# hidayetersindursun/LangSplatV2

Measured on AMD Instinct MI355X. Metric: frames/s fwd+bwd @ 1M Gaussians 1080p 3+16ch; achieved HBM GB/s, higher is better.
Workload: dtype f32; 1 GPU; BASELINE cfg3: 1M Gaussians, 1920x1080, SH deg 3 + 16 dense language channels, fwd+bwd, all inputs require grad; 1 view per GPU; gaussians=1000000, width=1920, height=1080, lang_dim=16, sh_degree=3, global_batch=1, parallelism=single GPU

## Files before the change

langsplatv2_amd/csrc/render_bwd.hip:

```cpp
#include "render_common.h"
#include "render_det.h"

#ifndef LSR_BWD_SPLAT_PF
#define LSR_BWD_SPLAT_PF 1
#endif
#ifndef LSR_BWD_LO_RREG
#define LSR_BWD_LO_RREG 1
#endif
#ifndef LSR_BWD16_WAVES
#define LSR_BWD16_WAVES 4
#endif
#ifndef LSR_MF_WAVES
#define LSR_MF_WAVES 2
#endif

namespace lsr {

#define LSR_ORD_NB 64
#ifndef LSR_ORD_THREADS
#define LSR_ORD_THREADS 1024
#endif
#define LSR_ORD_KPT 16
__global__ void __launch_bounds__(LSR_ORD_THREADS) k_bwd_order(const uint32_t* __restrict__ lcount,
                                                    const uint32_t* __restrict__ tile_start, int n,
                                                    uint4* __restrict__ border)
{
    __shared__ uint32_t cnt[LSR_ORD_NB];
    const int q = n / 8, r = n % 8, x = blockIdx.x;
    const int lo = x < r ? x * (q + 1) : r * (q + 1) + (x - r) * q;
    const int len = q + (x < r ? 1 : 0);
    const int tid = threadIdx.x;
    if (tid < LSR_ORD_NB) cnt[tid] = 0u;
    __syncthreads();
    auto key = [&](int i) { return min((int)((lcount[lo + i] + 15u) >> 4), LSR_ORD_NB - 1); };
    constexpr int STEP = LSR_ORD_THREADS * LSR_ORD_KPT;
    int kr[LSR_ORD_KPT];
    for (int c = 0; c < len; c += STEP) {
#pragma unroll
        for (int j = 0; j < LSR_ORD_KPT; j++) {
            const int i = c + tid + LSR_ORD_THREADS * j;
            kr[j] = i < len ? key(i) : -1;
        }
#pragma unroll
        for (int j = 0; j < LSR_ORD_KPT; j++)
            if (kr[j] >= 0) atomicAdd(&cnt[kr[j]], 1u);
    }
    __syncthreads();
    if (tid < 64) {
        static_assert(LSR_ORD_NB == 64, "one bucket per lane");
        const uint32_t v = cnt[63 - tid];
        uint32_t incl = v;
#pragma unroll
        for (int d = 1; d < 64; d <<= 1) {
            const uint32_t u = __shfl_up(incl, d, 64);
            if (tid >= d) incl += u;
        }
        cnt[63 - tid] = (uint32_t)lo + incl - v;
    }
    __syncthreads();
    for (int c = 0; c < len; c += STEP) {
        if (len > STEP) {
#pragma unroll
            for (int j = 0; j < LSR_ORD_KPT; j++) {
                const int i = c + tid + LSR_ORD_THREADS * j;
                kr[j] = i < len ? key(i) : -1;
            }
        }
#pragma unroll
        for (int j = 0; j < LSR_ORD_KPT; j++)
            if (kr[j] >= 0) {
                const uint32_t blk = (uint32_t)(lo + c + tid + LSR_ORD_THREADS * j);
                border[atomicAdd(&cnt[kr[j]], 1u)] =
                    make_uint4(blk, tile_start[blk >> 2], tile_start[(blk >> 2) + 1], lcount[blk]);
            }
    }
}

hipError_t launch_bwd_order(const RenderArgs& a, uint4* border, hipStream_t st)
{
    const int n = 4 * a.cam.gx * a.cam.gy;
    if (n == 0) return hipSuccess;
    k_bwd_order<<<8, LSR_ORD_THREADS, 0, st>>>(a.lcount, a.tile_start, n, border);
    return hipGetLastError();
}

int grad_row_width(int D)
{
    const int nl = lang_set_for(D);
    const int nv = LSR_GROW_LANG + (nl > 0 ? nl : 0);
    return (nv + 31) / 32 * 32;
}

template <int NL>
struct BwdFrags {
    static constexpr int C = 3 + NL;
    static constexpr int KS = (C + 3) / 4;
    static constexpr int NBC = (C + 15) / 16;
    float dotB[KS][4];
    float chB[NBC][16];
    float momB[16];
};

template <int NL>
__device__ __forceinline__ float gd_at(const RenderBwdArgs& b, int c, int q, int bx, int by)
{
    const Cam& cm = b.f.cam;
    const int qx = bx + (q & 7), qy = by + (q >> 3);
    const bool ok = qx < cm.W && qy < cm.H && c < 3 + b.f.D;
    const size_t HW = (size_t)cm.H * cm.W;
    const size_t pix = (size_t)min(qy, cm.H - 1) * cm.W + min(qx, cm.W - 1);
    const float* src = c < 3 ? b.dout_color + (size_t)c * HW : b.dout_lang + (size_t)min(c - 3, max(b.f.D - 1, 0)) * HW;
    if (c >= 3 && b.f.D == 0) src = b.dout_color;
    const float v = src[pix];
    return ok ? v : 0.f;
}

#ifndef LSR_GRP_STRIDE
#define LSR_GRP_STRIDE 66
#endif
#define LSR_BUF_OOB 0x7ffffffc
#define LSR_MOM9_STRIDE 12
#define LSR_LOG2E 1.4426950408889634f
#define LSR_MF_ATOMIC(ptr, v) atomicAdd((ptr), (v))

__device__ __forceinline__ uint64_t lanes_abs_lt(float v, float bound)
{
    uint64_t m;
    asm("v_cmp_gt_f32_e64 %0, %1, |%2|" : "=s"(m) : "s"(bound), "v"(v));
    return m;
}

struct WaveStageG {
    float4 A[80];
    float4 B[80];
    uint32_t gid[80];
};

#define LSR_LST_CHUNK 16
struct WaveStageL {
    float4 A[2 * LSR_LST_CHUNK];
    float4 B[2 * LSR_LST_CHUNK];
};
template <int NL, bool LD, bool LST, bool DET = false>
constexpr int bwd_waves() { return (LST && LD && NL == 16 && !DET) ? LSR_BWD16_WAVES : LSR_MF_WAVES; }

__device__ __forceinline__ void glds16(const void* g, const void* lds)
{
    const uint32_t l = (uint32_t)(uintptr_t)lds;
    uint32_t keep;
    asm volatile("s_mov_b32 %0, m0\n\ts_mov_b32 m0, %2\n\ts_nop 0\n\tglobal_load_lds_dwordx4 %1, off\n\ts_mov_b32 m0, %0"
                 : "=&s"(keep) : "v"(g), "s"(l) : "memory");
}

template <int N>
__device__ __forceinline__ void wait_vmcnt()
{
    static_assert(N >= 0 && N <= 63, "vmcnt is 6 bits");
    asm volatile("s_waitcnt vmcnt(%0)" ::"n"(N) : "memory");
}

__device__ __forceinline__ int stage_candidates_geo(WaveStageG& st, int carry, bool valid, uint32_t gid, int pos,
                                                    int bx, int by, const float4* __restrict__ splatA,
                                                    const float4* __restrict__ splatB)
{
    float4 A = make_float4(0.f, 0.f, 0.f, 0.f), B = A;
    if (valid) {
        A = splatA[gid];
        B = splatB[gid];
    }
    const bool ok = valid && block_overlap(A.x, A.y, __float_as_uint(B.w), bx, by) &&
                    block_overlap_exact(A.x, A.y, A.z, A.w, B.x, B.z, bx, by);
    const uint64_t m = wave_ballot(ok);
    if (ok) {
        const int r = carry + __builtin_amdgcn_mbcnt_hi((uint32_t)(m >> 32), __builtin_amdgcn_mbcnt_lo((uint32_t)m, 0u));
        st.A[r] = A;
        st.B[r] = make_float4(B.x, B.y, B.z, __int_as_float(pos));
        st.gid[r] = gid;
    }
    wave_lds_fence();
    return __popcll(m);
}

__device__ __forceinline__ int stage_candidates_geo_rec(WaveStageG& st, int carry, bool valid, uint32_t gid, int pos,
                                                        int bx, int by, float4 A, float4 B)
{
    const bool ok = valid && block_overlap(A.x, A.y, __float_as_uint(B.w), bx, by) &&
                    block_overlap_exact(A.x, A.y, A.z, A.w, B.x, B.z, bx, by);
    const uint64_t m = wave_ballot(ok);
    if (ok) {
        const int r = carry + __builtin_amdgcn_mbcnt_hi((uint32_t)(m >> 32), __builtin_amdgcn_mbcnt_lo((uint32_t)m, 0u));
        st.A[r] = A;
        st.B[r] = make_float4(B.x, B.y, B.z, __int_as_float(pos));
        st.gid[r] = gid;
    }
    wave_lds_fence();
    return __popcll(m);
}

template <int NL>
__device__ __forceinline__ float feature_at(const RenderArgs& a, uint32_t gid, int c)
{
    const bool ok = c < 3 + a.D;
    const float* src = c < 3 ? a.rgb + 3 * (size_t)gid + c
                             : (ok ? a.lang + (size_t)gid * a.D + (c - 3) : a.rgb + 3 * (size_t)gid);
    const float v = *src;
    return ok ? v : 0.f;
}

template <int NL, bool VEC>
__device__ __forceinline__ int dot_channel(int t, int lg)
{
    if constexpr (VEC) {
        if (t < NL / 4) return 3 + 16 * (t >> 2) + 4 * lg + (t & 3);
        return lg < 3 ? lg : 3 + NL;
    }
    return 4 * t + lg;
}

template <int NL, bool VEC, int KS>
__device__ __forceinline__ void dot_features(const RenderArgs& a, uint32_t gid, int lg, float (&af)[KS])
{
    if constexpr (VEC) {
        static_assert(NL % 16 == 0 && KS == NL / 4 + 1, "VEC: whole 16-channel lines");
        const float4* row = reinterpret_cast<const float4*>(a.lang) + (size_t)gid * (NL / 4) + lg;
#pragma unroll
        for (int r = 0; r < NL / 16; r++) {
            const float4 v = row[4 * r];
            af[4 * r + 0] = v.x;
            af[4 * r + 1] = v.y;
            af[4 * r + 2] = v.z;
            af[4 * r + 3] = v.w;
        }
        const float c = a.rgb[3 * (size_t)gid + min(lg, 2)];
        af[NL / 4] = lg < 3 ? c : 0.f;
    } else {
#pragma unroll
        for (int t = 0; t < KS; t++) af[t] = feature_at<NL>(a, gid, 4 * t + lg);
    }
}

#define BWD_MFMA(a, b_, c) __builtin_amdgcn_mfma_f32_16x16x4f32((a), (b_), (c), 0, 0, 0)


template <int NL, bool LO = false, bool LD = false, bool SP = false, bool LST = false, bool DET = false>
__global__ void __launch_bounds__(64) __attribute__((amdgpu_waves_per_eu(bwd_waves<NL, LD, LST, DET>()))) k_render_bwd_mf(RenderBwdArgs b)
{
    static_assert(!(LST && SP), "the sparse-input backward follows the quick forward (no lists)");
    static_assert(!(DET && SP), "the deterministic backward expands the sparse input (lsr_api backward_quick)");
    static_assert(!LO || NL > 0, "language-only backward needs D > 0");
    static_assert(!SP || LO, "the sparse-input gradient is a language-only backward");
    static_assert(!LD || (!LO && NL % 16 == 0), "direct dL/dlang needs whole 16-channel lines");
    using FR = BwdFrags<NL>;
    constexpr int KS = FR::KS;
    constexpr bool VEC = LD;
    constexpr bool RREG = LD || (LO && !SP && LSR_BWD_LO_RREG);
    constexpr int NBC = (NL + 15) / 16;
    constexpr int NBA = NBC > 0 ? NBC : 1;
    __shared__ float2 sRG[64];
    __shared__ float sBc[64];
    constexpr int GS = LSR_GRP_STRIDE;
    __shared__ std::conditional_t<LST, WaveStageL, WaveStageG> stv;
    auto& st = stv;
    auto& stl = stv;
    constexpr int GCOL0 = LO ? 0 : (LD ? 16 : LSR_GROW_LANG);
    constexpr int GRL = (GCOL0 + NL + 15) / 16;
    constexpr int GRS = 16 * GRL + 4;
    constexpr int DUG = (16 * GS > 16 * GRS) ? 16 * GS : 16 * GRS;
    __shared__ float sDU[DUG];
    __shared__ __attribute__((aligned(16))) float sAT[16 * GS];
    static_assert(16 * LSR_MOM9_STRIDE <= 16 * GS, "moment rows must fit the aT tile");
    float* const sGr = sDU;
    float* const sMom = sAT;

    const RenderArgs& a = b.f;
    const Cam& c = a.cam;
    const WaveTile wt(a, LST ? a.border : nullptr);
    const int lane = threadIdx.x;
    const int lg = lane >> 4, li = lane & 15;
    const PixMap pm(c, wt.tile, lane + (wt.sub << 6));
    const bool inside = pm.px < c.W && pm.py < c.H;
    const float pfx = (float)pm.px, pfy = (float)pm.py;
    const float cx = (float)pm.bx + 3.5f, cy = (float)pm.by + 3.5f;
    const uint32_t rs = wt.ent ? wt.rs : a.tile_start[wt.tile];
    const size_t HW = (size_t)c.H * c.W;
    const size_t pix = (size_t)pm.py * c.W + pm.px;
    const int D = a.D;
    const int VP = b.VP;
    const float ddelx_dx = 0.5f * (float)c.W, ddely_dy = 0.5f * (float)c.H;
    const uint64_t nbg = (uint64_t)a.P * (uint64_t)VP * 4u;
    const uint64_t nbl = LD ? (uint64_t)a.P * (uint64_t)D * 4u : 0u;
    const bool buf_atom = nbg < (uint64_t)LSR_BUF_OOB && nbl < (uint64_t)LSR_BUF_OOB;
    const __amdgpu_buffer_rsrc_t rg =
        __builtin_amdgcn_make_buffer_rsrc(b.grad_acc, 0, (int)min(nbg, (uint64_t)LSR_BUF_OOB), 0x00020000);
    const __amdgpu_buffer_rsrc_t rl = __builtin_amdgcn_make_buffer_rsrc(
        LD ? b.lang_acc : b.grad_acc, 0, (int)min(LD ? nbl : nbg, (uint64_t)LSR_BUF_OOB), 0x00020000);

    const float T_final = inside ? a.final_T[pix] : 0.f;
    const int last = inside ? (int)a.n_contrib[pix] : 0;
    const int wmax = wave_max_i(last);
    if (wmax == 0) return;
    constexpr bool SPF = LSR_BWD_SPLAT_PF && NL <= 32;
    auto pl_at = [&](int q) -> uint32_t { const uint32_t v = a.point_list[rs + max(q, 0)]; return q >= 0 ? v : 0u; };
    uint32_t gid1 = 0u, gid2 = 0u;
    float4 A1 = make_float4(0.f, 0.f, 0.f, 0.f), B1 = A1;
    const uint32_t lcnt = LST ? (wt.ent ? wt.lc : a.lcount[4 * wt.tile + wt.sub]) : 0u;
    const size_t lbase = LST ? (size_t)4 * rs + (size_t)wt.sub * ((wt.ent ? wt.re : a.tile_start[wt.tile + 1]) - rs) : 0;
    if constexpr (!LST) {
        gid1 = pl_at(wmax - 1 - lane);
        if constexpr (SPF) {
            gid2 = pl_at(wmax - 65 - lane);
            A1 = a.splatA[gid1];
            B1 = a.splatB[gid1];
        }
        for (int e = lane; e < 80; e += 64) {
            st.A[e] = make_float4(0.f, 0.f, 0.f, 0.f);
            st.B[e] = make_float4(0.f, 0.f, 0.f, __int_as_float(0x7fffffff));
            st.gid[e] = 0u;
        }
    }
    auto list_dma = [&](int c0, int off) {
        const int e = (int)lcnt - 1 - (c0 + lane);
        const size_t src = lbase + (size_t)(e >= 0 ? e : 0);
        if (lane < LSR_LST_CHUNK) {
            glds16(a.listA + src, stl.A + off);
            glds16(a.listB + src, stl.B + off);
        }
    };

    float dr0 = 0.f, dr1 = 0.f, dr2 = 0.f;
    if constexpr (!LO) {
        dr0 = gd_at<NL>(b, 0, lane, pm.bx, pm.by);
        dr1 = gd_at<NL>(b, 1, lane, pm.bx, pm.by);
        dr2 = gd_at<NL>(b, 2, lane, pm.bx, pm.by);
    }
    float dotB[KS][4], chB[NBA][16];
    const uint64_t HW4 = (uint64_t)HW * 4u;
    const bool gd_buf = VEC && HW4 * (uint64_t)(D > 3 ? D : 3) < 0x7fffffffull;
    if (VEC && gd_buf) {
        const __amdgpu_buffer_rsrc_t rcol = __builtin_amdgcn_make_buffer_rsrc((void*)b.dout_color, 0, (int)(HW4 * 3u), 0x00020000);
        const __amdgpu_buffer_rsrc_t rlng = __builtin_amdgcn_make_buffer_rsrc((void*)b.dout_lang, 0, (int)(HW4 * (uint64_t)D), 0x00020000);
        const uint32_t hw4 = (uint32_t)HW4;
        auto poff = [&](int q) -> uint32_t {
            const int qx = pm.bx + (q & 7), qy = pm.by + (q >> 3);
            return (qx < c.W && qy < c.H) ? (uint32_t)(qy * c.W + qx) * 4u : 0x80000000u;
        };
        auto ld = [&](__amdgpu_buffer_rsrc_t r, uint32_t off) {
            return __builtin_bit_cast(float, __builtin_amdgcn_raw_buffer_load_b32(r, off, 0, 0));
        };
        uint32_t pa[4];
#pragma unroll
        for (int pb = 0; pb < 4; pb++) pa[pb] = poff(pb * 16 + li);
#pragma unroll
        for (int t = 0; t < KS; t++)
#pragma unroll
            for (int pb = 0; pb < 4; pb++) {
                if (t < NL / 4) {
                    const int chl = dot_channel<NL, VEC>(t, lg) - 3;
                    dotB[t][pb] = ld(rlng, (uint32_t)chl * hw4 + pa[pb]);
                } else {
                    dotB[t][pb] = ld(rcol, lg < 3 ? (uint32_t)lg * hw4 + pa[pb] : 0x80000000u);
                }
            }
#pragma unroll
        for (int nb = 0; nb < NBC; nb++)
#pragma unroll
            for (int t = 0; t < 16; t++) chB[nb][t] = ld(rlng, (uint32_t)(nb * 16 + li) * hw4 + poff(4 * t + lg));
    } else
    {
    if constexpr (!LO) {
#pragma unroll
        for (int t = 0; t < KS; t++)
#pragma unroll
            for (int pb = 0; pb < 4; pb++)
                dotB[t][pb] = gd_at<NL>(b, dot_channel<NL, VEC>(t, lg), pb * 16 + li, pm.bx, pm.by);
    }
#pragma unroll
    for (int nb = 0; nb < NBC; nb++)
#pragma unroll
        for (int t = 0; t < 16; t++)
            chB[nb][t] = gd_at<NL>(b, 3 + nb * 16 + li, 4 * t + lg, pm.bx, pm.by);
    }
    const float lxe = (float)lg - 3.5f, lxo = (float)lg + 0.5f;
    const float lxe2 = lxe * lxe, lxo2 = lxo * lxo;
    const float bg0 = c.bg[0], bg1 = c.bg[1], bg2 = c.bg[2];
    const float bg_dot = LO ? 0.f : bg0 * dr0 + bg1 * dr1 + bg2 * dr2;

    const bool has_bg = (bg0 != 0.f) || (bg1 != 0.f) || (bg2 != 0.f);
    float T = T_final;
    float S = 0.f;

    int carry = 0;
    float af[KS];
    if constexpr (!LO) {
        sRG[lane] = make_float2(dr0, dr1);
        sBc[lane] = dr2;
    }
    constexpr int ATOMICS_PER_GROUP = GRL * 4;
    constexpr int OPG = ATOMICS_PER_GROUP;
    constexpr int CGR = LSR_LST_CHUNK / 16;
    constexpr int CHUNK_OPS = CGR * OPG < 63 ? CGR * OPG : 63;
    constexpr int CH = LST ? LSR_LST_CHUNK : 64;
    if constexpr (LST) list_dma(0, 0);
    const int cend = LST ? (int)lcnt : wmax;
    for (int c0 = 0; c0 < cend; c0 += CH) {
        int n, nfull;
        const float4* SA;
        const float4* SB;
        const uint32_t* SG;
        if constexpr (LST) {
            const int off = (c0 / CH & 1) * CH;
            if (c0 == 0 || !buf_atom || DET) wait_vmcnt<0>();
            else wait_vmcnt<CHUNK_OPS>();
            if (c0 + CH < cend) list_dma(c0 + CH, CH - off);
            n = nfull = min(CH, cend - c0);
            SA = stl.A + off;
            SB = stl.B + off;
            SG = reinterpret_cast<const uint32_t*>(stl.B + off) + 2;
        } else {
            const int p = wmax - 1 - (c0 + lane);
            const bool valid = p >= 0;
            if constexpr (SPF) {
                const uint32_t gid = gid1;
                const float4 Ac = A1, Bc = B1;
                gid1 = gid2;
                A1 = a.splatA[gid1];
                B1 = a.splatB[gid1];
                gid2 = pl_at(p - 128);
                n = carry + stage_candidates_geo_rec(st, carry, valid, gid, p, pm.bx, pm.by, Ac, Bc);
            } else {
                const uint32_t gid = gid1;
                gid1 = pl_at(p - 64);
                n = carry + stage_candidates_geo(st, carry, valid, gid, p, pm.bx, pm.by, a.splatA, a.splatB);
            }
            nfull = (c0 + 64 >= wmax) ? n : (n & ~15);
            SA = st.A;
            SB = st.B;
            SG = st.gid;
        }
        constexpr int SGS = LST ? 4 : 1;

        for (int g0 = 0; g0 < nfull; g0 += 16) {
            const int kn = min(16, nfull - g0);
            if constexpr (!LO) {
                const uint32_t gi = SG[SGS * (g0 + (li < kn ? li : 0))];
                dot_features<NL, VEC>(a, gi, lg, af);
            }
            uint64_t near_m = 0u;
            const int kn_u = __builtin_amdgcn_readfirstlane(kn);
            const int opl = __float_as_int(SB[g0 + li].y);
#define BWD_OP(k) __int_as_float(__builtin_amdgcn_readlane(opl, (k)))
            float Gr[16];
            (void)Gr;
#pragma unroll
            for (int k = 0; k < 16; k++) {
                const float4 A = SA[g0 + k];
                const float4 B = SB[g0 + k];
                const float power = splat_power(A.z, A.w, B.x, A.x - pfx, A.y - pfy);
                const bool cj = (k < kn_u) && (__float_as_int(B.w) < last) && !(power > 0.0f);
                const float G = cj ? __builtin_amdgcn_exp2f(power * LSR_LOG2E) : 0.f;
                const float d = fminf(0.99f, B.y * G) - (1.0f / 255.0f);
                near_m |= lanes_abs_lt(d, 2e-8f);
                Gr[k] = d >= 0.f ? G : 0.f;
            }
            if (near_m != 0u) {
#pragma unroll
                for (int k = 0; k < 16; k++) {
                    if (k >= kn) break;
                    const int j = g0 + k;
                    const float4 A = SA[j];
                    const float4 B = SB[j];
                    const float power = splat_power(A.z, A.w, B.x, A.x - pfx, A.y - pfy);
                    const bool cj = (__float_as_int(B.w) < last) & !(power > 0.0f) & (LST || !(power < B.z));
                    const float af2 = fminf(0.99f, B.y * __builtin_amdgcn_exp2f(power * LSR_LOG2E));
                    if (cj & (fabsf(af2 - (1.0f / 255.0f)) < 2e-8f)) {
                        const float G = expf_det(power);
                        const float alpha = fminf(0.99f, B.y * G);
                        Gr[k] = !(alpha < 1.0f / 255.0f) ? G : 0.f;
                    }
                }
            }
            float dv[16];
            (void)dv;
            if constexpr (!LO) {
                f32x4 acc[4];
#pragma unroll
                for (int pb = 0; pb < 4; pb++) acc[pb] = f32x4{0.f, 0.f, 0.f, 0.f};
#pragma unroll
                for (int t = 0; t < KS; t++)
#pragma unroll
                    for (int pb = 0; pb < 4; pb++)
                        acc[pb] = BWD_MFMA(af[t], dotB[t][pb], acc[pb]);
#pragma unroll
                for (int r = 0; r < 4; r++) {
                    uint32_t x0 = __float_as_uint(acc[0][r]), x1 = __float_as_uint(acc[1][r]);
                    uint32_t x2 = __float_as_uint(acc[2][r]), x3 = __float_as_uint(acc[3][r]);
                    auto s02 = __builtin_amdgcn_permlane32_swap(x0, x2, false, false);
                    auto s13 = __builtin_amdgcn_permlane32_swap(x1, x3, false, false);
                    auto s01 = __builtin_amdgcn_permlane16_swap(s02[0], s13[0], false, false);
                    auto s23 = __builtin_amdgcn_permlane16_swap(s02[1], s13[1], false, false);
                    dv[0 + r] = __uint_as_float(s01[0]);
                    dv[4 + r] = __uint_as_float(s01[1]);
                    dv[8 + r] = __uint_as_float(s23[0]);
                    dv[12 + r] = __uint_as_float(s23[1]);
                }
            }
            wave_lds_fence();
            if constexpr (LO) {
#pragma unroll
                for (int k = 0; k < 16; k++) {
                    const float G = Gr[k];
                    const float al = fminf(0.99f, BWD_OP(k) * G);
                    T = T * __builtin_amdgcn_rcpf(1.f - al);
                    sAT[k * GS + lane] = al * T;
                }
            } else if (has_bg) {
#pragma unroll
                for (int k = 0; k < 16; k++) {
                    const float G = Gr[k];
                    const float dot = dv[k];
                    const float al = fminf(0.99f, BWD_OP(k) * G);
                    const float om = 1.f - al;
                    const float rcp = __builtin_amdgcn_rcpf(om);
                    T = T * rcp;
                    const float dL_dalpha = fmaf(-T_final * rcp, bg_dot, (dot - S) * T);
                    sDU[k * GS + lane] = dL_dalpha * G;
                    sAT[k * GS + lane] = al * T;
                    S = fmaf(al, dot, om * S);
                }
            } else {
#pragma unroll
                for (int k = 0; k < 16; k++) {
                    const float G = Gr[k];
                    const float dot = dv[k];
                    const float al = fminf(0.99f, BWD_OP(k) * G);
                    const float om = 1.f - al;
                    T = T * __builtin_amdgcn_rcpf(om);
                    sDU[k * GS + lane] = ((dot - S) * T) * G;
                    sAT[k * GS + lane] = al * T;
                    S = fmaf(al, dot, om * S);
                }
            }
            wave_lds_fence();
            f32x4 ch[NBA];
#pragma unroll
            for (int nb = 0; nb < NBA; nb++) ch[nb] = f32x4{0.f, 0.f, 0.f, 0.f};
            float M0 = 0.f, M1 = 0.f, M2 = 0.f, M3 = 0.f, M4 = 0.f, M5 = 0.f;
            float C0 = 0.f, C1 = 0.f, C2 = 0.f;
            float ue = 0.f;
            if constexpr (LO) {
#pragma unroll
                for (int t = 0; t < 16; t++) {
                    const float aa = sAT[li * GS + 4 * t + lg];
#pragma unroll
                    for (int nb = 0; nb < NBC; nb++) ch[nb] = BWD_MFMA(aa, chB[nb][t], ch[nb]);
                }
            } else {
#pragma unroll
            for (int t = 0; t < 16; t++) {
                const float au = sDU[li * GS + 4 * t + lg];
                const float aa = sAT[li * GS + 4 * t + lg];
#pragma unroll
                for (int nb = 0; nb < NBC; nb++) ch[nb] = BWD_MFMA(aa, chB[nb][t], ch[nb]);
                const float2 rg = sRG[4 * t + lg];
                const float4 d = make_float4(rg.x, rg.y, sBc[4 * t + lg], 0.f);
                C0 = fmaf(aa, d.x, C0);
                C1 = fmaf(aa, d.y, C1);
                C2 = fmaf(aa, d.z, C2);
                const float ly = (float)(t >> 1) - 3.5f;
                if ((t & 1) == 0) {
                    M0 += au;
                    M2 = fmaf(ly, au, M2);
                    M5 = fmaf(ly * ly, au, M5);
                } else {
                    M1 += au;
                    M3 = fmaf(ly, au, M3);
                    M4 = fmaf(ly * ly, au, M4);
                }
            }
            {
                const float se = M0, so = M1, ye = M2, yo = M3, qe = M5, qo = M4;
                M0 = se + so;
                M1 = fmaf(lxe, se, lxo * so);
                M2 = ye + yo;
                M3 = fmaf(lxe2, se, lxo2 * so);
                M4 = fmaf(lxe, ye, lxo * yo);
                M5 = qe + qo;
            }
            {
                auto red32 = [](float x, float y) {
                    const auto r = __builtin_amdgcn_permlane32_swap(__float_as_uint(x), __float_as_uint(y), false, false);
                    return __uint_as_float(r[0]) + __uint_as_float(r[1]);
                };
                auto red16 = [](float x, float y) {
                    const auto r = __builtin_amdgcn_permlane16_swap(__float_as_uint(x), __float_as_uint(y), false, false);
                    return __uint_as_float(r[0]) + __uint_as_float(r[1]);
                };
                const float Y0 = red16(red32(M0, M1), red32(M2, M3));
                const float Y1 = red16(red32(M4, M5), red32(C0, C1));
                const float X4 = red32(C2, C2);
                const float Y2 = red16(X4, X4);
                const int s0 = ((lg & 1) << 1) | (lg >> 1);
                float* const mr = sMom + li * LSR_MOM9_STRIDE;
                mr[s0] = Y0;
                mr[4 + s0] = Y1;
                if (lg == 0) mr[8] = Y2;
            }
            }
#pragma unroll
            for (int nb = 0; nb < (RREG ? 0 : NBC); nb++) {
                const int chn = nb * 16 + li;
                if (chn < NL) {
#pragma unroll
                    for (int r = 0; r < 4; r++) sGr[(4 * lg + r) * GRS + GCOL0 + chn] = ch[nb][r];
                }
            }
            if constexpr (!LO) wave_lds_fence();
            if (!LO && lane < kn) {
                const int j = g0 + lane;
                const float4 A = SA[j];
                const float4 B = SB[j];
                const float* const mr = sMom + lane * LSR_MOM9_STRIDE;
                const float4 m03 = *reinterpret_cast<const float4*>(mr);
                const float4 m47 = *reinterpret_cast<const float4*>(mr + 4);
                const float S0 = m03.x, S1 = m03.y, S2 = m03.z, S3 = m03.w, S4 = m47.x, S5 = m47.y;
                C0 = m47.z;
                C1 = m47.w;
                C2 = mr[8];
                const float X = A.x - cx, Y = A.y - cy;
                const float Sdx = fmaf(X, S0, -S1), Sdy = fmaf(Y, S0, -S2);
                const float Sdxx = fmaf(X, fmaf(X, S0, -2.f * S1), S3);
                const float Sdxy = fmaf(X, fmaf(Y, S0, -S2), fmaf(-Y, S1, S4));
                const float Sdyy = fmaf(Y, fmaf(Y, S0, -2.f * S2), S5);
                const float o = B.y;
                float* gr = sGr + lane * GRS;
                gr[0] = -o * ddelx_dx * fmaf(A.z, Sdx, A.w * Sdy);
                gr[1] = -o * ddely_dy * fmaf(B.x, Sdy, A.w * Sdx);
                gr[2] = -0.5f * o * Sdxx;
                gr[3] = -o * Sdxy;
                gr[4] = -0.5f * o * Sdyy;
                gr[5] = S0;
                gr[6] = C0;
                gr[7] = C1;
                gr[8] = C2;
            }
            wave_lds_fence();
            if constexpr (SP) {
                const int K = a.K;
                for (int e = lane; e < 16 * K; e += 64) {
                    const int slot = e / K, m = e - slot * K;
                    if (slot < kn) {
                        const size_t off = (size_t)SG[SGS * (g0 + slot)] * K + m;
                        const int q = quick_index(a.qi, a.qidx_dtype, off);
                        if (q >= 0 && q < D) {
                            const float v = sGr[slot * GRS + GCOL0 + q];
                            if (v != 0.f) LSR_MF_ATOMIC(b.qw_acc + off, v);
                        }
                    }
                }
            } else {
                uint32_t gq[4];
                float vq[GRL][4];
                auto slot_of = [&](int q) { return RREG ? 4 * lg + q : 4 * q + lg; };
#pragma unroll
                for (int q = 0; q < 4; q++) gq[q] = SG[SGS * (g0 + slot_of(q))];
#pragma unroll
                for (int h = 0; h < GRL; h++)
#pragma unroll
                    for (int q = 0; q < 4; q++) {
                        if (RREG && LO)
                            vq[h][q] = ch[h][q];
                        else if (RREG && h > 0)
                            vq[h][q] = ch[h - 1][q];
                        else
                            vq[h][q] = sGr[slot_of(q) * GRS + 16 * h + li];
                    }
                if constexpr (DET) {
                    uint32_t* const dflag = reinterpret_cast<uint32_t*>(b.det_bounds + 2);
                    uint32_t sq[4];
#pragma unroll
                    for (int q = 0; q < 4; q++) sq[q] = slot_of(q) < kn ? b.det_sh[gq[q]] : 0u;
#pragma unroll
                    for (int h = 0; h < GRL; h++) {
                        const int f = 16 * h + li;
                        const bool fcol = LO ? (f < D)
                                          : LD ? (h == 0 ? (f < 9) : (f - 16 < D))
                                               : ((f < 9) | ((f >= LSR_GROW_LANG) & (f < LSR_GROW_LANG + D)));
                        const int cls = LO ? 0 : ((LD && h > 0) ? 0 : det_class_of(f));
#pragma unroll
                        for (int q = 0; q < 4; q++) {
                            const float v = vq[h][q];
                            if (fcol & (slot_of(q) < kn) & (v != 0.f)) {
                                const int sh = (int)(int8_t)(sq[q] >> (8 * cls));
                                if (LD && h > 0)
                                    det_add(b.det_lang + (size_t)gq[q] * D + (f - 16), v, sh, dflag);
                                else
                                    det_add(b.det_rows + (size_t)gq[q] * VP + f, v, sh, dflag);
                            }
                        }
                    }
                } else if (buf_atom) {
                    static_assert(ATOMICS_PER_GROUP == GRL * 4, "the LST wait counts these atomics");
#pragma unroll
                    for (int h = 0; h < GRL; h++) {
                        const int f = 16 * h + li;
                        const bool fcol = LO ? (f < D)
                                          : LD ? (h == 0 ? (f < 9) : (f - 16 < D))
                                               : ((f < 9) | ((f >= LSR_GROW_LANG) & (f < LSR_GROW_LANG + D)));
#pragma unroll
                        for (int q = 0; q < 4; q++) {
                            const float v = vq[h][q];
                            const bool on = fcol & (slot_of(q) < kn) & (v != 0.f);
                            if (LD && h > 0) {
                                const int off = (int)(gq[q] * (uint32_t)D + (uint32_t)(f - 16)) * 4;
                                __builtin_amdgcn_raw_ptr_buffer_atomic_fadd_f32(v, rl, on ? off : LSR_BUF_OOB, 0, 0);
                            } else {
                                const int off = (int)(gq[q] * (uint32_t)VP + (uint32_t)f) * 4;
                                __builtin_amdgcn_raw_ptr_buffer_atomic_fadd_f32(v, rg, on ? off : LSR_BUF_OOB, 0, 0);
                            }
                        }
                    }
                } else
#pragma unroll
                for (int h = 0; h < GRL; h++) {
                    const int f = 16 * h + li;
                    const bool fcol = LO ? (f < D)
                                      : LD ? (h == 0 ? (f < 9) : (f - 16 < D))
                                           : ((f < 9) | ((f >= LSR_GROW_LANG) & (f < LSR_GROW_LANG + D)));
#pragma unroll
                    for (int q = 0; q < 4; q++) {
                        const float v = vq[h][q];
                        if (fcol & (slot_of(q) < kn) & (v != 0.f)) {
                            if (LD && h > 0)
                                LSR_MF_ATOMIC(b.lang_acc + (size_t)gq[q] * D + (f - 16), v);
                            else
                                LSR_MF_ATOMIC(b.grad_acc + (size_t)gq[q] * VP + f, v);
                        }
                    }
                }
            }
            wave_lds_fence();
        }
        if constexpr (!LST) {
            carry = n - nfull;
            if (nfull > 0 && lane < carry) {
                st.A[lane] = st.A[nfull + lane];
                st.B[lane] = st.B[nfull + lane];
                st.gid[lane] = st.gid[nfull + lane];
            }
        }
        wave_lds_fence();
    }
}


using BwdKernel = void (*)(RenderBwdArgs);

hipError_t launch_render_bwd_lang(const RenderBwdArgs& b, hipStream_t st)
{
    const int T = b.f.cam.gx * b.f.cam.gy;
    if (T == 0) return hipSuccess;
    if (b.det_rows && (!b.det_bounds || !b.det_sh)) return hipErrorInvalidValue;
    BwdKernel k = nullptr;
    const bool known = with_lang_set<4>(lang_set_for(b.f.D), [&](auto nl) {
        constexpr int NL = decltype(nl)::value;
        with_bools([&](auto lst, auto det) { k = k_render_bwd_mf<NL, true, false, false, lst.value, det.value>; },
                   b.f.listA != nullptr, b.det_rows != nullptr);
    });
    if (!known) return hipErrorInvalidValue;
    k<<<4 * T, 64, 0, st>>>(b);
    return hipGetLastError();
}

hipError_t launch_render_bwd_lang_sparse(const RenderBwdArgs& b, hipStream_t st)
{
    const int T = b.f.cam.gx * b.f.cam.gy;
    if (T == 0) return hipSuccess;
    if (!b.qw_acc || !b.f.qi || b.f.K <= 0) return hipErrorInvalidValue;
    BwdKernel k = nullptr;
    const bool known = with_lang_set<4>(lang_set_for(b.f.D), [&](auto nl) {
        k = k_render_bwd_mf<decltype(nl)::value, true, false, true>;
    });
    if (!known) return hipErrorInvalidValue;
    k<<<4 * T, 64, 0, st>>>(b);
    return hipGetLastError();
}

static constexpr bool lang_direct_set(int D) { return D == 16 || D == 32; }
bool bwd_lang_direct(int D)
{
    return lang_direct_set(D);
}

hipError_t launch_render_bwd(const RenderBwdArgs& b, hipStream_t st)
{
    const int T = b.f.cam.gx * b.f.cam.gy;
    if (T == 0) return hipSuccess;
    const bool lst = b.f.listA != nullptr;
    const bool det = b.det_rows != nullptr;
    const bool ld = b.lang_acc != nullptr;
    if (det && (!b.det_bounds || !b.det_sh || (ld != (b.det_lang != nullptr)))) return hipErrorInvalidValue;
    if (ld && (!bwd_lang_direct(b.f.D) || (uintptr_t)b.f.lang % 16 != 0)) return hipErrorInvalidValue;
    BwdKernel k = nullptr;
    const bool known = with_lang_set(lang_set_for(b.f.D), [&](auto nl) {
        constexpr int NL = decltype(nl)::value;
        with_bools([&](auto ldc, auto lstc, auto detc) {
            if constexpr (!ldc.value || lang_direct_set(NL))
                k = k_render_bwd_mf<NL, false, ldc.value, false, lstc.value, detc.value>;
        }, ld, lst, det);
    });
    if (!known) return hipErrorInvalidValue;
    k<<<4 * T, 64, 0, st>>>(b);
    return hipGetLastError();
}

}
```

langsplatv2_amd/csrc/render_fwd.hip:

```cpp
#include "render_common.h"

namespace lsr {

template <int NL, int F4>
__device__ __forceinline__ void stage_features(float4* dst, const float* rgb, const float* lang, int D, uint32_t gid)
{
    float row[F4 * 4];
    row[0] = rgb[3 * gid];
    row[1] = rgb[3 * gid + 1];
    row[2] = rgb[3 * gid + 2];
    if (NL > 0 && D == NL && (NL % 4) == 0) {
        const float4* src = reinterpret_cast<const float4*>(lang + (size_t)gid * NL);
#pragma unroll
        for (int q = 0; q < NL / 4; q++) {
            const float4 v = src[q];
            row[3 + 4 * q] = v.x; row[4 + 4 * q] = v.y; row[5 + 4 * q] = v.z; row[6 + 4 * q] = v.w;
        }
    } else {
#pragma unroll
        for (int k = 0; k < NL; k++) row[3 + k] = (k < D) ? lang[(size_t)gid * D + k] : 0.f;
    }
#pragma unroll
    for (int k = 3 + NL; k < F4 * 4; k++) row[k] = 0.f;
#pragma unroll
    for (int q = 0; q < F4; q++) dst[q] = make_float4(row[4 * q], row[4 * q + 1], row[4 * q + 2], row[4 * q + 3]);
}

template <int NL>
constexpr bool fwd_ml = NL >= 16;
template <int F4, bool SF>
struct WaveStageP {
    static constexpr int NE = SF ? 68 : 64;
    f32x2 X[NE / 2], Y[NE / 2], CA[NE / 2], CB[NE / 2], CC[NE / 2], OP[NE / 2];
    float4 F[SF ? 1 : 64 * F4];
    uint32_t gid[SF ? NE : 1];
    float4 R[SF ? NE : 1];
    uint32_t pos[SF ? NE : 1];
    uint8_t src[SF ? 1 : 64];
};

struct ListSink {
    float4* A = nullptr;
    float4* B = nullptr;
    uint32_t pos = 0;
};

template <int NL, int F4, bool LST = false>
__device__ __forceinline__ int stage_candidates_p_rec(WaveStageP<F4, fwd_ml<NL>>& st, bool valid, uint32_t gid,
                                                      int pos, int bx, int by, float4 A, float4 B,
                                                      const float* __restrict__ rgb, const float* __restrict__ lang,
                                                      int D, const ListSink& ls = ListSink(), uint64_t* mo = nullptr,
                                                      int off = 0)
{
    constexpr bool SF = fwd_ml<NL>;
    constexpr int NE = WaveStageP<F4, SF>::NE;
    const bool ok = valid && block_overlap(A.x, A.y, __float_as_uint(B.w), bx, by) &&
                    block_overlap_exact(A.x, A.y, A.z, A.w, B.x, B.z, bx, by);
    const uint64_t m = wave_ballot(ok);
    const int cnt = __popcll(m);
    if constexpr (LST) *mo = m;
    if (ok) {
        const int r = __builtin_amdgcn_mbcnt_hi((uint32_t)(m >> 32), __builtin_amdgcn_mbcnt_lo((uint32_t)m, 0u));
        if constexpr (LST) {
            if (ls.A) {
                ls.A[ls.pos + r] = A;
                ls.B[ls.pos + r] = make_float4(B.x, B.y, __uint_as_float(gid), __int_as_float(pos - 1));
            }
        }
        const int i = off + r;
        float* base = reinterpret_cast<float*>(&st) + (i & 1);
        const int e = (i >> 1) * 2;
        base[0 * NE + e] = A.x;
        base[1 * NE + e] = A.y;
        base[2 * NE + e] = A.z;
        base[3 * NE + e] = A.w;
        base[4 * NE + e] = B.x;
        base[5 * NE + e] = B.y;
        if constexpr (SF) {
            st.pos[i] = (uint32_t)pos;
            st.gid[i] = gid;
            st.R[i] = make_float4(rgb[3 * (size_t)gid], rgb[3 * (size_t)gid + 1], rgb[3 * (size_t)gid + 2], 0.f);
        } else {
            st.src[r] = (uint8_t)(threadIdx.x & 63);
        }
        if constexpr (!SF)
            stage_features<NL, F4>(&st.F[r * F4], rgb, lang, D, gid);
    }
    wave_lds_fence();
    return cnt;
}

template <int NL, int F4, bool LST = false>
__device__ __forceinline__ int stage_candidates_p(WaveStageP<F4, fwd_ml<NL>>& st, bool valid, uint32_t gid, int pos, int bx,
                                                  int by, const float4* __restrict__ splatA,
                                                  const float4* __restrict__ splatB, const float* __restrict__ rgb,
                                                  const float* __restrict__ lang, int D, const ListSink& ls = ListSink(),
                                                  uint64_t* mo = nullptr, int off = 0)
{
    float4 A = make_float4(0.f, 0.f, 0.f, 0.f), B = A;
    if (valid) {
        A = splatA[gid];
        B = splatB[gid];
    }
    return stage_candidates_p_rec<NL, F4, LST>(st, valid, gid, pos, bx, by, A, B, rgb, lang, D, ls, mo, off);
}

__device__ __forceinline__ void zero_backward_accumulators(const RenderArgs& a)
{
    typedef float v4f __attribute__((ext_vector_type(4)));
    const size_t stride = (size_t)gridDim.x * 64;
    if (a.zero) {
        v4f* const z = reinterpret_cast<v4f*>(a.zero);
        for (size_t i = (size_t)blockIdx.x * 64 + threadIdx.x; i < a.zero_n16; i += stride)
            __builtin_nontemporal_store(v4f{0.f, 0.f, 0.f, 0.f}, z + i);
    }
    if (a.zero2) {
        v4f* const z = reinterpret_cast<v4f*>(a.zero2);
        for (size_t i = (size_t)blockIdx.x * 64 + threadIdx.x; i < a.zero2_n16; i += stride)
            __builtin_nontemporal_store(v4f{0.f, 0.f, 0.f, 0.f}, z + i);
    }
}

template <int NL, bool ML>
constexpr int fwd_waves() { return (ML && NL == 16) ? 6 : 1; }
template <int NL, bool ZERO = false, bool ML = false, bool MLM = false>
__global__ void __launch_bounds__(64) __attribute__((amdgpu_waves_per_eu(fwd_waves<NL, ML>()))) k_render_fwd(RenderArgs a)
{
    if constexpr (ZERO) zero_backward_accumulators(a);
    constexpr int C = 3 + NL;
    constexpr int F4 = (C + 3) / 4;
    constexpr bool SF = fwd_ml<NL>;
    static_assert(!ML || NL == 16 || NL == 32 || NL == 64, "ML: whole 16-channel language blocks");
    static_assert(ML == SF, "the ML form and the SF stage go together (NL >= 16)");
    constexpr int MLB = ML ? NL / 16 : 1;
    __shared__ WaveStageP<F4, SF> st;

    const Cam& c = a.cam;
    const WaveTile wt(a);
    const int lane = threadIdx.x;
    const PixMap pm(c, wt.tile, lane + (wt.sub << 6));
    const bool inside = pm.px < c.W && pm.py < c.H;
    const float pfx = (float)pm.px, pfy = (float)pm.py;
    const uint32_t rs = a.tile_start[wt.tile], re = a.tile_start[wt.tile + 1];
    const int D = (ML && !MLM) ? NL : a.D;

    float T = 1.0f;
    bool done = !inside;
    float acc[F4 * 4];
#pragma unroll
    for (int k = 0; k < F4 * 4; k++) acc[k] = 0.f;
    f32x4 mlacc[MLB][4];
#pragma unroll
    for (int nb = 0; nb < MLB; nb++)
#pragma unroll
        for (int pb = 0; pb < 4; pb++) mlacc[nb][pb] = f32x4{0.f, 0.f, 0.f, 0.f};
    uint32_t last = 0;

    ListSink ls;
    uint32_t nst = 0, nlast = 0, blast = rs;
    uint64_t mlast = 0;
    if constexpr (ZERO) {
        if (a.listA) {
            ls.A = a.listA + (size_t)4 * rs + (size_t)wt.sub * (re - rs);
            ls.B = a.listB + (size_t)4 * rs + (size_t)wt.sub * (re - rs);
        }
    }
    uint32_t next_gid = (rs + lane < re) ? a.point_list[rs + lane] : 0u;
    constexpr bool FSPF = !SF;
    uint32_t next_gid2 = 0u;
    float4 A1 = make_float4(0.f, 0.f, 0.f, 0.f), B1 = A1;
    if (FSPF && rs < re) {
        next_gid2 = (rs + 64 + lane < re) ? a.point_list[rs + 64 + lane] : 0u;
        A1 = a.splatA[next_gid];
        B1 = a.splatB[next_gid];
    }
    int carry = 0;
    for (uint32_t base = rs; base < re; base += 64) {
        if (wave_ballot(!done) == 0) break;
        const uint32_t idx = base + lane;
        const bool valid = idx < re;
        const uint32_t gid = next_gid;
        int n;
        uint64_t mchunk = 0;
        ls.pos = nst;
        if constexpr (FSPF) {
            const float4 Ac = A1, Bc = B1;
            n = stage_candidates_p_rec<NL, F4, ZERO>(st, valid, gid, (int)(idx - rs) + 1, pm.bx, pm.by, Ac, Bc, a.rgb,
                                                     a.lang, D, ls, &mchunk, ML ? carry : 0);
            next_gid = next_gid2;
            A1 = a.splatA[next_gid];
            B1 = a.splatB[next_gid];
            const uint32_t q = min(idx + 128, re - 1);
            const uint32_t v = a.point_list[q];
            next_gid2 = idx + 128 < re ? v : 0u;
        } else {
            next_gid = (idx + 64 < re) ? a.point_list[idx + 64] : 0u;
            n = stage_candidates_p<NL, F4, ZERO>(st, valid, gid, (int)(idx - rs) + 1, pm.bx, pm.by, a.splatA,
                                                 a.splatB, a.rgb, a.lang, D, ls, &mchunk, ML ? carry : 0);
        }
        if constexpr (ZERO) {
            mlast = mchunk;
            nlast = nst;
            blast = base;
            nst += (uint32_t)n;
        }
        int lastj = -1;
        if constexpr (ML) {
            const int lg = lane >> 4, li = lane & 15;
            const float* const Fs = reinterpret_cast<const float*>(st.F);
            n += carry;
            const int nproc = (base + 64 >= re) ? n : (n & ~3);
            int q0 = 0;
            for (; q0 < nproc; q0 += 4) {
                if (wave_ballot(!done) == 0) break;
                float av[MLB];
#pragma unroll
                for (int nb = 0; nb < MLB; nb++) {
                    const int ch = 16 * nb + li;
                    float fa;
                    if constexpr (SF)
                        fa = a.lang[(size_t)st.gid[min(q0 + lg, n - 1)] * D + (MLM ? min(ch, D - 1) : ch)];
                    else
                        fa = Fs[(q0 + lg) * (F4 * 4) + 3 + ch];
                    av[nb] = ((q0 + lg < n) & (!MLM || ch < D)) ? fa : 0.f;
                }
                float al[4];
                bool cm[4];
#pragma unroll
                for (int h = 0; h < 2; h++) {
                    const int j0 = q0 + 2 * h, e = j0 >> 1;
                    const f32x2 sX = st.X[e], sY = st.Y[e], sCA = st.CA[e], sCB = st.CB[e], sCC = st.CC[e];
                    const f32x2 OP = st.OP[e];
                    const f32x2 dx = sX - f32x2{pfx, pfx}, dy = sY - f32x2{pfy, pfy};
                    const f32x2 P = __builtin_elementwise_fma(f32x2{-0.5f, -0.5f},
                                                              __builtin_elementwise_fma(sCA * dx, dx, (sCC * dy) * dy),
                                                              -((sCB * dx) * dy));
                    const f32x2 EX = expf_det2(P);
                    const float a0 = fminf(0.99f, OP.x * EX.x), a1 = fminf(0.99f, OP.y * EX.y);
                    const bool c0 = (j0 < n) & !done & !(P.x > 0.0f) & !(a0 < 1.0f / 255.0f);
                    const bool c1 = (j0 + 1 < n) & !done & !(P.y > 0.0f) & !(a1 < 1.0f / 255.0f);
                    al[2 * h] = c0 ? a0 : 0.f;
                    al[2 * h + 1] = c1 ? a1 : 0.f;
                    cm[2 * h] = c0;
                    cm[2 * h + 1] = c1;
                }
                float s4[4];
                auto rgb_of = [&](int k) -> float3 {
                    const int kk = min(q0 + k, n - 1);
                    if constexpr (SF) {
                        const float4 f = st.R[kk];
                        return make_float3(f.x, f.y, f.z);
                    } else {
                        const float4 f = st.F[kk * F4];
                        return make_float3(f.x, f.y, f.z);
                    }
                };
                float Tk[5];
                Tk[0] = T;
#pragma unroll
                for (int k = 0; k < 4; k++) Tk[k + 1] = Tk[k] * (1.0f - al[k]);
                if (wave_ballot(Tk[4] < 0.0001f) == 0u) {
#pragma unroll
                    for (int k = 0; k < 4; k++) {
                        const float aT = al[k] * Tk[k];
                        const float3 f = rgb_of(k);
                        acc[0] = fmaf(f.x, aT, acc[0]);
                        acc[1] = fmaf(f.y, aT, acc[1]);
                        acc[2] = fmaf(f.z, aT, acc[2]);
                        lastj = cm[k] ? q0 + k : lastj;
                        s4[k] = aT;
                    }
                    T = Tk[4];
                } else {
#pragma unroll
                    for (int k = 0; k < 4; k++) {
                        const float alk = al[k];
                        const float test_T = T * (1.0f - alk);
                        const bool ok0 = (alk != 0.f) & !done;
                        const bool term = ok0 & (test_T < 0.0001f);
                        done = done | term;
                        const bool ok = ok0 & !term;
                        const float aT = ok ? alk * T : 0.f;
                        const float3 f = rgb_of(k);
                        acc[0] = fmaf(f.x, aT, acc[0]);
                        acc[1] = fmaf(f.y, aT, acc[1]);
                        acc[2] = fmaf(f.z, aT, acc[2]);
                        T = ok ? test_T : T;
                        lastj = ok ? q0 + k : lastj;
                        s4[k] = aT;
                    }
                }
                {
                    auto sw32 = [](float& x, float& y) {
                        const auto r = __builtin_amdgcn_permlane32_swap(__float_as_uint(x), __float_as_uint(y), false, false);
                        x = __uint_as_float(r[0]);
                        y = __uint_as_float(r[1]);
                    };
                    auto sw16 = [](float& x, float& y) {
                        const auto r = __builtin_amdgcn_permlane16_swap(__float_as_uint(x), __float_as_uint(y), false, false);
                        x = __uint_as_float(r[0]);
                        y = __uint_as_float(r[1]);
                    };
                    sw32(s4[0], s4[2]);
                    sw32(s4[1], s4[3]);
                    sw16(s4[0], s4[1]);
                    sw16(s4[2], s4[3]);
                }
#pragma unroll
                for (int pb = 0; pb < 4; pb++)
#pragma unroll
                    for (int nb = 0; nb < MLB; nb++)
                        mlacc[nb][pb] = __builtin_amdgcn_mfma_f32_16x16x4f32(av[nb], s4[pb], mlacc[nb][pb], 0, 0, 0);
            }
            if constexpr (SF) {
                if (lastj >= 0) last = st.pos[lastj];
                lastj = -1;
                carry = n - q0;
                if (q0 > 0 && carry > 0) {
                    if (lane < carry) {
                        const int i = q0 + lane;
                        float* fb = reinterpret_cast<float*>(&st);
                        constexpr int NE = WaveStageP<F4, SF>::NE;
                        float v[6];
#pragma unroll
                        for (int f = 0; f < 6; f++) v[f] = fb[f * NE + i];
                        const uint32_t pv = st.pos[i], gv = st.gid[i];
                        const float4 rv = st.R[i];
#pragma unroll
                        for (int f = 0; f < 6; f++) fb[f * NE + lane] = v[f];
                        st.pos[lane] = pv;
                        st.gid[lane] = gv;
                        st.R[lane] = rv;
                    }
                }
            }
        } else
        for (int j0 = 0; j0 < n; j0 += 2) {
            if (wave_ballot(!done) == 0) break;
            const bool two = j0 + 1 < n;
            const int j1 = two ? j0 + 1 : j0;
            const int e = j0 >> 1;
            const f32x2 sX = st.X[e], sY = st.Y[e], sCA = st.CA[e], sCB = st.CB[e], sCC = st.CC[e];
            const f32x2 OP = st.OP[e];
            const f32x2 dx = sX - f32x2{pfx, pfx}, dy = sY - f32x2{pfy, pfy};
            const f32x2 P = __builtin_elementwise_fma(f32x2{-0.5f, -0.5f},
                                                      __builtin_elementwise_fma(sCA * dx, dx, (sCC * dy) * dy),
                                                      -((sCB * dx) * dy));
            const float p0 = P.x, p1 = P.y;
            bool ok0 = !done && !(p0 > 0.0f);
            bool ok1 = two && !done && !(p1 > 0.0f);
            const f32x2 EX = expf_det2(P);
            const float al0 = fminf(0.99f, OP.x * EX.x);
            const float al1 = fminf(0.99f, OP.y * EX.y);
            ok0 = ok0 && !(al0 < 1.0f / 255.0f);
            ok1 = ok1 && !(al1 < 1.0f / 255.0f);
            {
                const float test_T = T * (1.0f - al0);
                const bool term = ok0 && (test_T < 0.0001f);
                done = done || term;
                ok0 = ok0 && !term;
                ok1 = ok1 && !term;
                const float aT = ok0 ? al0 * T : 0.f;
                {
#pragma unroll
                    for (int f = 0; f < F4; f++) {
                        const float4 v = st.F[j0 * F4 + f];
                        if (4 * f + 0 < C) acc[4 * f + 0] = fmaf(v.x, aT, acc[4 * f + 0]);
                        if (4 * f + 1 < C) acc[4 * f + 1] = fmaf(v.y, aT, acc[4 * f + 1]);
                        if (4 * f + 2 < C) acc[4 * f + 2] = fmaf(v.z, aT, acc[4 * f + 2]);
                        if (4 * f + 3 < C) acc[4 * f + 3] = fmaf(v.w, aT, acc[4 * f + 3]);
                        else asm volatile("" ::"v"(v.w));
                    }
                }
                T = ok0 ? test_T : T;
                lastj = ok0 ? j0 : lastj;
            }
            {
                const float test_T = T * (1.0f - al1);
                const bool term = ok1 && (test_T < 0.0001f);
                done = done || term;
                ok1 = ok1 && !term;
                const float aT = ok1 ? al1 * T : 0.f;
                {
#pragma unroll
                    for (int f = 0; f < F4; f++) {
                        const float4 v = st.F[j1 * F4 + f];
                        if (4 * f + 0 < C) acc[4 * f + 0] = fmaf(v.x, aT, acc[4 * f + 0]);
                        if (4 * f + 1 < C) acc[4 * f + 1] = fmaf(v.y, aT, acc[4 * f + 1]);
                        if (4 * f + 2 < C) acc[4 * f + 2] = fmaf(v.z, aT, acc[4 * f + 2]);
                        if (4 * f + 3 < C) acc[4 * f + 3] = fmaf(v.w, aT, acc[4 * f + 3]);
                        else asm volatile("" ::"v"(v.w));
                    }
                }
                T = ok1 ? test_T : T;
                lastj = ok1 ? j1 : lastj;
            }
        }
        if constexpr (!ML) {
            if (lastj >= 0) last = (uint32_t)(base - rs) + 1u + st.src[lastj];
        }
        wave_lds_fence();
    }
    if constexpr (ZERO) {
        if (a.listA) {
            const int wmax = wave_max_i(inside ? (int)last : 0);
            const int off = wmax - (int)(blast - rs);
            uint32_t cnt = nlast;
            if (off > 0) cnt += (uint32_t)__popcll(off >= 64 ? mlast : (mlast & ((1ull << off) - 1ull)));
            if (lane == 0) a.lcount[4 * wt.tile + wt.sub] = cnt;
        }
    }
    if (inside) {
        const size_t HW = (size_t)c.H * c.W;
        const size_t pix = (size_t)pm.py * c.W + pm.px;
        a.final_T[pix] = T;
        a.n_contrib[pix] = last;
#pragma unroll
        for (int ch = 0; ch < 3; ch++) a.out_color[ch * HW + pix] = fmaf(T, c.bg[ch], acc[ch]);
        if constexpr (!ML) {
#pragma unroll
            for (int k = 0; k < NL; k++)
                if (k < D) a.out_lang[k * HW + pix] = acc[3 + k];
        }
    }
    if constexpr (ML) {
        const size_t HW = (size_t)c.H * c.W;
        const int lg = lane >> 4, li = lane & 15;
#pragma unroll
        for (int pb = 0; pb < 4; pb++) {
            const int q = pb * 16 + li;
            const int qx = pm.bx + (q & 7), qy = pm.by + (q >> 3);
            if (qx < c.W && qy < c.H) {
                const size_t pix = (size_t)qy * c.W + qx;
#pragma unroll
                for (int nb = 0; nb < MLB; nb++)
#pragma unroll
                    for (int r = 0; r < 4; r++)
                        if (16 * nb + 4 * lg + r < D) a.out_lang[(size_t)(16 * nb + 4 * lg + r) * HW + pix] = mlacc[nb][pb][r];
            }
        }
    }
}

int lang_set_for(int D)
{
    return lang_set_ceil(LangSets{}, D);
}

hipError_t launch_render_fwd(const RenderArgs& a, hipStream_t st)
{
    const int T = a.cam.gx * a.cam.gy;
    if (T == 0) return hipSuccess;
    if (a.qw) return launch_render_fwd_quick(a, st);
    void (*k)(RenderArgs) = nullptr;
    const bool known = with_lang_set(lang_set_for(a.D), [&](auto nl) {
        constexpr int NL = decltype(nl)::value;
        constexpr bool ML = fwd_ml<NL>;
        with_bools([&](auto zero, auto mlm) {
            if constexpr (ML || !mlm.value) k = k_render_fwd<NL, zero.value, ML, mlm.value>;
        }, a.zero || a.zero2, ML && a.D != NL);
    });
    if (!known) return hipErrorInvalidValue;
    k<<<4 * T, 64, 0, st>>>(a);
    return hipGetLastError();
}

}
```

Measured before the change: 952.5 frames/s.

## Specialize direct-lang backward with static strides and add fused four-wide exp in forward

In the backward kernel with direct language gradients, the channel count and gradient stride become compile-time constants. A new template flag picks buffer atomics at launch time and drops the fallback global-atomic path, which is meant to cut address arithmetic and code size. In the forward kernel, the exponentials for four Gaussians are computed in one interleaved vector routine, and empty asm statements are added to steer register allocation and instruction scheduling. The launcher now rejects any gradient stride other than 16 when direct language gradients are used, which narrows the supported inputs.

After: 962.5 frames/s (median of 6 runs). 1.1% higher.

```diff
diff --git a/langsplatv2_amd/csrc/render_bwd.hip b/langsplatv2_amd/csrc/render_bwd.hip
--- a/langsplatv2_amd/csrc/render_bwd.hip
+++ b/langsplatv2_amd/csrc/render_bwd.hip
@@ -9,6 +9,9 @@
 #endif
 #ifndef LSR_BWD16_WAVES
 #define LSR_BWD16_WAVES 4
+#endif
+#ifndef LSR_BWD_LD_STATIC
+#define LSR_BWD_LD_STATIC 1
 #endif
 #ifndef LSR_MF_WAVES
 #define LSR_MF_WAVES 2
@@ -242,9 +245,10 @@
 #define BWD_MFMA(a, b_, c) __builtin_amdgcn_mfma_f32_16x16x4f32((a), (b_), (c), 0, 0, 0)
 
 
-template <int NL, bool LO = false, bool LD = false, bool SP = false, bool LST = false, bool DET = false>
+template <int NL, bool LO = false, bool LD = false, bool SP = false, bool LST = false, bool DET = false, bool BA = false>
 __global__ void __launch_bounds__(64) __attribute__((amdgpu_waves_per_eu(bwd_waves<NL, LD, LST, DET>()))) k_render_bwd_mf(RenderBwdArgs b)
 {
+    static_assert(!BA || (LD && !DET), "BA: the direct-dL/dlang float-atomic backward");
     static_assert(!(LST && SP), "the sparse-input backward follows the quick forward (no lists)");
     static_assert(!(DET && SP), "the deterministic backward expands the sparse input (lsr_api backward_quick)");
     static_assert(!LO || NL > 0, "language-only backward needs D > 0");
@@ -284,12 +288,12 @@
     const uint32_t rs = wt.ent ? wt.rs : a.tile_start[wt.tile];
     const size_t HW = (size_t)c.H * c.W;
     const size_t pix = (size_t)pm.py * c.W + pm.px;
-    const int D = a.D;
-    const int VP = b.VP;
+    const int D = (LD && LSR_BWD_LD_STATIC) ? NL : a.D;
+    const int VP = (LD && LSR_BWD_LD_STATIC) ? 16 : b.VP;
     const float ddelx_dx = 0.5f * (float)c.W, ddely_dy = 0.5f * (float)c.H;
     const uint64_t nbg = (uint64_t)a.P * (uint64_t)VP * 4u;
     const uint64_t nbl = LD ? (uint64_t)a.P * (uint64_t)D * 4u : 0u;
-    const bool buf_atom = nbg < (uint64_t)LSR_BUF_OOB && nbl < (uint64_t)LSR_BUF_OOB;
+    const bool buf_atom = BA || (nbg < (uint64_t)LSR_BUF_OOB && nbl < (uint64_t)LSR_BUF_OOB);
     const __amdgpu_buffer_rsrc_t rg =
         __builtin_amdgcn_make_buffer_rsrc(b.grad_acc, 0, (int)min(nbg, (uint64_t)LSR_BUF_OOB), 0x00020000);
     const __amdgpu_buffer_rsrc_t rl = __builtin_amdgcn_make_buffer_rsrc(
@@ -719,7 +723,7 @@
                             }
                         }
                     }
-                } else
+                } else if constexpr (!BA)
 #pragma unroll
                 for (int h = 0; h < GRL; h++) {
                     const int f = 16 * h + li;
@@ -800,11 +804,17 @@
     const bool ld = b.lang_acc != nullptr;
     if (det && (!b.det_bounds || !b.det_sh || (ld != (b.det_lang != nullptr)))) return hipErrorInvalidValue;
     if (ld && (!bwd_lang_direct(b.f.D) || (uintptr_t)b.f.lang % 16 != 0)) return hipErrorInvalidValue;
+    if (ld && LSR_BWD_LD_STATIC && b.VP != 16) return hipErrorInvalidValue;
     BwdKernel k = nullptr;
     const bool known = with_lang_set(lang_set_for(b.f.D), [&](auto nl) {
         constexpr int NL = decltype(nl)::value;
         with_bools([&](auto ldc, auto lstc, auto detc) {
-            if constexpr (!ldc.value || lang_direct_set(NL))
+            if constexpr (ldc.value && !detc.value && LSR_BWD_LD_STATIC) {
+                const uint64_t nb = (uint64_t)b.f.P * (uint64_t)(NL > 16 ? NL : 16) * 4u;
+                if constexpr (lang_direct_set(NL))
+                    k = nb < (uint64_t)LSR_BUF_OOB ? k_render_bwd_mf<NL, false, true, false, lstc.value, false, true>
+                                                   : k_render_bwd_mf<NL, false, true, false, lstc.value, false>;
+            } else if constexpr (!ldc.value || lang_direct_set(NL))
                 k = k_render_bwd_mf<NL, false, ldc.value, false, lstc.value, detc.value>;
         }, ld, lst, det);
     });
diff --git a/langsplatv2_amd/csrc/render_fwd.hip b/langsplatv2_amd/csrc/render_fwd.hip
--- a/langsplatv2_amd/csrc/render_fwd.hip
+++ b/langsplatv2_amd/csrc/render_fwd.hip
@@ -1,6 +1,39 @@
 #include "render_common.h"
 
+#ifndef LSR_FWD_EXP4
+#define LSR_FWD_EXP4 1
+#endif
+#ifndef LSR_FWD_RGB
+#define LSR_FWD_RGB 1
+#endif
+
 namespace lsr {
+
+__device__ __forceinline__ void expf_det2x2(f32x2 x0, f32x2 x1, f32x2& e0, f32x2& e1)
+{
+    typedef uint32_t u32x2 __attribute__((ext_vector_type(2)));
+    auto fma2 = [](f32x2 a, f32x2 b, f32x2 c) { return __builtin_elementwise_fma(a, b, c); };
+    auto k2 = [](float v) { return f32x2{v, v}; };
+    x0 = f32x2{__builtin_amdgcn_fmed3f(x0.x, -87.0f, 1.0e30f), __builtin_amdgcn_fmed3f(x0.y, -87.0f, 1.0e30f)};
+    x1 = f32x2{__builtin_amdgcn_fmed3f(x1.x, -87.0f, 1.0e30f), __builtin_amdgcn_fmed3f(x1.y, -87.0f, 1.0e30f)};
+    const f32x2 t0 = fma2(x0, k2(1.44269504088896341f), k2(12582912.0f));
+    const f32x2 t1 = fma2(x1, k2(1.44269504088896341f), k2(12582912.0f));
+    const f32x2 n0 = t0 - k2(12582912.0f), n1 = t1 - k2(12582912.0f);
+    f32x2 r0 = fma2(n0, k2(-0.693145751953125f), x0), r1 = fma2(n1, k2(-0.693145751953125f), x1);
+    r0 = fma2(n0, k2(-1.428606765330187e-06f), r0);
+    r1 = fma2(n1, k2(-1.428606765330187e-06f), r1);
+    f32x2 p0 = k2(0x1.6aea1ap-10f), p1 = p0;
+    constexpr float cf[6] = {0x1.1267d2p-7f, 0x1.555820p-5f, 0x1.555418p-3f, 0x1.fffffcp-2f, 1.0f, 1.0f};
+#pragma unroll
+    for (int i = 0; i < 6; i++) {
+        p0 = fma2(p0, r0, k2(cf[i]));
+        p1 = fma2(p1, r1, k2(cf[i]));
+    }
+    const u32x2 s0 = (__builtin_bit_cast(u32x2, t0) << 23) + u32x2{0x3f800000u, 0x3f800000u};
+    const u32x2 s1 = (__builtin_bit_cast(u32x2, t1) << 23) + u32x2{0x3f800000u, 0x3f800000u};
+    e0 = p0 * __builtin_bit_cast(f32x2, s0);
+    e1 = p1 * __builtin_bit_cast(f32x2, s1);
+}
 
 template <int NL, int F4>
 __device__ __forceinline__ void stage_features(float4* dst, const float* rgb, const float* lang, int D, uint32_t gid)
@@ -226,6 +259,20 @@
                 }
                 float al[4];
                 bool cm[4];
+                f32x2 EX4[2];
+                (void)EX4;
+                if constexpr (LSR_FWD_EXP4) {
+                    f32x2 P4[2];
+#pragma unroll
+                    for (int h = 0; h < 2; h++) {
+                        const int e = (q0 >> 1) + h;
+                        const f32x2 dx = st.X[e] - f32x2{pfx, pfx}, dy = st.Y[e] - f32x2{pfy, pfy};
+                        P4[h] = __builtin_elementwise_fma(f32x2{-0.5f, -0.5f},
+                                                          __builtin_elementwise_fma(st.CA[e] * dx, dx, (st.CC[e] * dy) * dy),
+                                                          -((st.CB[e] * dx) * dy));
+                    }
+                    expf_det2x2(P4[0], P4[1], EX4[0], EX4[1]);
+                }
 #pragma unroll
                 for (int h = 0; h < 2; h++) {
                     const int j0 = q0 + 2 * h, e = j0 >> 1;
@@ -235,7 +282,7 @@
                     const f32x2 P = __builtin_elementwise_fma(f32x2{-0.5f, -0.5f},
                                                               __builtin_elementwise_fma(sCA * dx, dx, (sCC * dy) * dy),
                                                               -((sCB * dx) * dy));
-                    const f32x2 EX = expf_det2(P);
+                    const f32x2 EX = LSR_FWD_EXP4 ? EX4[h] : expf_det2(P);
                     const float a0 = fminf(0.99f, OP.x * EX.x), a1 = fminf(0.99f, OP.y * EX.y);
                     const bool c0 = (j0 < n) & !done & !(P.x > 0.0f) & !(a0 < 1.0f / 255.0f);
                     const bool c1 = (j0 + 1 < n) & !done & !(P.y > 0.0f) & !(a1 < 1.0f / 255.0f);
@@ -249,6 +296,7 @@
                     const int kk = min(q0 + k, n - 1);
                     if constexpr (SF) {
                         const float4 f = st.R[kk];
+                        if constexpr (LSR_FWD_RGB) asm volatile("" ::"v"(f.w));
                         return make_float3(f.x, f.y, f.z);
                     } else {
                         const float4 f = st.F[kk * F4];
@@ -267,6 +315,7 @@
                         acc[0] = fmaf(f.x, aT, acc[0]);
                         acc[1] = fmaf(f.y, aT, acc[1]);
                         acc[2] = fmaf(f.z, aT, acc[2]);
+                        if constexpr (LSR_FWD_RGB) asm("" : "+v"(acc[1]), "+v"(acc[2]));
                         lastj = cm[k] ? q0 + k : lastj;
                         s4[k] = aT;
                     }
```
